# The-African-Research-Collective/karanta-ocr

Hardware: AMD Instinct MI355X
Metric: pages_per_sec (higher is better)
Workload: dtype bf16; 1 GPU; Qwen2-VL-2B bf16 greedy, batch=8 synthetic 1024x1024 pages per GPU, max_pixels=1003520 (grid 70x70, 1225 image tokens), prompt P=1394 tokens, T_out=1024 (ignore_eos), random-init weights; global_batch=8, parallelism=dp1, decode=hipGraph replay

## Files before the change

karanta_ocr_amd/_lib.py:

```python
from __future__ import annotations

import ctypes as C
import os
from typing import Optional

_HERE = os.path.dirname(os.path.abspath(__file__))
LIB_PATH = os.path.join(_HERE, "libkaranta_hip.so")

c_p = C.c_void_p
i32, i64, f32 = C.c_int, C.c_int64, C.c_float


class KarantaHipError(RuntimeError):
    pass


SIGNATURES = {
    "kr_version": [],
    "kr_last_error": [],
    "kr_device_info": [i32, C.c_char_p, C.POINTER(i32), C.POINTER(C.c_size_t)],
    "kr_set_device": [i32],
    "kr_stream_synchronize": [c_p],
    "kr_stream_create_cu_mask": [C.POINTER(c_p), i32],
    "kr_stream_create_cu_range": [C.POINTER(c_p), i32, i32],
# ... 94 lines not shown
    return C.byref(NarrowOpts(zero_ptr or None, int(zero_bytes), 1 if atomic_out else 0, int(part_rows)))

class Dec32(C.Structure):
    _fields_ = [("xp", c_p), ("w_packed", c_p), ("w_scale", c_p), ("bias", c_p), ("residual", c_p), ("ldr", C.c_int64),
                ("out", c_p), ("out_f32", c_p), ("ldc", C.c_int64), ("M", C.c_int32), ("N", C.c_int32), ("K", C.c_int32),
                ("waves_ref", C.c_int32), ("ksplit", C.c_int32), ("atomic_out", C.c_int32), ("tiles_per_wg", C.c_int32),
                ("group_split", C.c_int32), ("reserved0", C.c_int32), ("zero_ptr", c_p), ("zero_bytes", C.c_uint64),
                ("cs_table", c_p), ("cs_stride", C.c_int32), ("prompt_len", c_p), ("ctx_len", c_p),
                ("q_out", c_p), ("kcache", c_p), ("vtcache", c_p), ("heads", C.c_int32), ("kv_heads", C.c_int32), ("s_max", C.c_int32)]


ABI_MAJOR = 4
DEC_OUT_XP = 0x100
ADJ_CAP = 320
EPI_NONE, EPI_QUICK_GELU, EPI_GELU_ERF, EPI_SILU_MUL, EPI_SILU_MUL8 = 0, 1, 2, 3, 4
DEC_PLAIN, DEC_SILU, DEC_ROPE_KV, DEC_ARGMAX, DEC_SILU8 = 0, 1, 2, 3, 4


class _Lib:
    def __init__(self, path: str):
        if not os.path.exists(path):
            raise KarantaHipError(
                f"{path} not found: build it with `python -m karanta_ocr_amd.build` "
                "(the MI355X engine has no CPU fallback)")
        import torch

        try:
            self._dll = C.CDLL(path, mode=C.RTLD_GLOBAL)
        except OSError as e:
            raise KarantaHipError(f"cannot load {path}: {e}") from e
        self.path = path
        for name, argtypes in SIGNATURES.items():
            try:
                fn = getattr(self._dll, name)
            except AttributeError as e:
                raise KarantaHipError(f"{path} does not export {name}") from e
            fn.argtypes = argtypes
            fn.restype = _RESTYPES.get(name, C.c_int)
            if name in ("kr_version", "kr_last_error"):
                setattr(self, name, fn)
            else:
                setattr(self, name, self._checked(name, fn))
        if self.kr_version() // 100 != ABI_MAJOR:
            raise KarantaHipError(f"{path} reports kr_version() = {self.kr_version()}, this binding is written against ABI major "
                                  f"{ABI_MAJOR} (include/karanta_hip.h): rebuild with `python -m karanta_ocr_amd.build`")
        self.experiments = hasattr(self._dll, "kr_oproj_heads")
        for name, argtypes in EXPERIMENT_SIGNATURES.items():
            if self.experiments:
                fn = getattr(self._dll, name)
                fn.argtypes, fn.restype = argtypes, C.c_int
                setattr(self, name, self._checked(name, fn))
            else:
                setattr(self, name, self._absent(name))

    @staticmethod
    def _absent(name):
        def call(*_):
            raise KarantaHipError(f"{name} is an experiment entry point (include/karanta_hip_experiments.h): this library was built "
                                  "without -DKR_EXPERIMENTS (csrc/tools/build_variant.py; load it through KARANTA_HIP_LIB)")
        call.__name__ = name
        return call

    def _checked(self, name, fn):
        def call(*args):
            rc = fn(*args)
            if rc != 0:
                msg = self._dll.kr_last_error()
                raise KarantaHipError(f"{name} -> {rc}: {msg.decode() if msg else ''}")
            return rc

        call.__name__ = name
        call.raw = fn
        return call


_LIB: Optional[_Lib] = None


def lib() -> _Lib:
    global _LIB
    if _LIB is None:
        _LIB = _Lib(os.environ.get("KARANTA_HIP_LIB", LIB_PATH))
    return _LIB


def ptr(t) -> int:
    return 0 if t is None else t.data_ptr()
```

karanta_ocr_amd/csrc/kr_decode.hip:

```cpp
#include "kr_decode_common.h"

namespace {

struct DecLinArgs {
    const kr_bf16* x; int64_t ldx;
    const kr_bf16* wp;
    const kr_bf16* bias;
    const kr_bf16* norm_w; float norm_eps;
    const kr_bf16* residual; int64_t ldr;
    kr_bf16* out; float* out_f32; int64_t ldc;
    int M, N, K, ksplit;
    int groups;
    float* ws; int* counters;
    const float* attn_ws; int attn_split;
    int xmode;
    const float* cs_table;
    const int32_t* prompt_len; int cs_stride;
    const int32_t* ctx_len;
    kr_bf16* q_out; kr_bf16* kcache; kr_bf16* vtcache;
    int heads, kv_heads, s_max;
    float* amax_val; int32_t* amax_idx;
    int wide_blocks, wide_waves;
    const float* part_in; kr_bf16* x_out; int64_t ldxo;
    const float* w_scale;
    float* x_out_f32; int64_t ldxf;
    kr_bf16* wide_x_out; int64_t wide_ldxo;
    int x_is_f32;
    const char* pf_ptr; int64_t pf_bytes; int pf_blocks;
    int part_rows;
    int n_part;
    int part_atomic;
    float* zero_ptr; int zero_n16;
    int out_xp;
};

template <int NT, int EPI, int WAVES>
__global__ void __launch_bounds__(WAVES * 64) dec_linear_kernel(const DecLinArgs a) {
    extern __shared__ __attribute__((aligned(16))) char smem[];
    constexpr int U = (WAVES == 16 ? 4 : 8) / NT;
    constexpr int NTHR = WAVES * 64;
    const int tid = threadIdx.x, lane = tid & 63;
    const int wave = __builtin_amdgcn_readfirstlane(tid >> 6);
    const int fr = lane & 15, fg = lane >> 4;
    const int ks = blockIdx.y;
    const int M = a.M, K = a.K;
    const int nchunks = K >> 6, ntiles = a.N >> 4;
    const int cpb = (nchunks + a.ksplit - 1) / a.ksplit;
    const int cb0 = min(ks * cpb, nchunks), cb1 = min(cb0 + cpb, nchunks);
    const int nblk = cb1 - cb0;
    const int per = (nblk + WAVES - 1) / WAVES;
    const int c0 = min(cb0 + wave * per, cb1), c1 = min(c0 + per, cb1);

    int tile[NT];
    const kr_bf16* wp[NT];
    bf16x8 wbuf[U][NT][2];
    auto set_item = [&](int g) {
        if (EPI == DEPI_ROPE_KV) {
            tile[0] = (g >> 2) * 8 + (g & 3);
            tile[NT - 1] = tile[0] + 4;
        } else {
#pragma unroll
            for (int t = 0; t < NT; ++t) tile[t] = g * NT + t;
        }
#pragma unroll
        for (int t = 0; t < NT; ++t) {
            const int tt = tile[t] < ntiles ? tile[t] : ntiles - 1;
            wp[t] = a.wp + ((int64_t)tt * nchunks) * 1024 + lane * 8;
        }
#pragma unroll
        for (int u = 0; u < U; ++u) {
            const int c = c0 + u;
            if (c < c1) {
#pragma unroll
                for (int t = 0; t < NT; ++t) {
                    wbuf[u][t][0] = ld8_nt(wp[t] + (int64_t)c * 1024);
                    wbuf[u][t][1] = ld8_nt(wp[t] + (int64_t)c * 1024 + 512);
                }
            }
        }
    };
    int g = blockIdx.x;
    set_item(g);

    const bool xlds = a.xmode != 0;
    const int xrow = nblk * 128 + 16;
    float* red = reinterpret_cast<float*>(smem + (xlds ? ((M * xrow + 127) & ~127) : 0));
// ... 801 lines not shown
        KR_CHECK_ARG(tiles_per_wave <= 5, "kr_linear_decode_wide: %d tiles over %d x %d waves is more than 5 tiles per wave", a.N >> 4,
                     blocks, waves);
        KR_CHECK_ARG(!a.x_is_f32 && !a.bias && !a.residual, "kr_linear_decode_wide: K-halves take bf16 x, no bias / residual");
        const size_t lds = (size_t)32 * (28 * 64 * 2 + 16);
        auto fn = tiles_per_wave <= 2 ? &dec_wide_kh_kernel<EPI, W8, true> : &dec_wide_kh_kernel<EPI, W8, false>;
        static KrPerDeviceOnce attr;
        if (attr.need()) {
            KR_CHECK_HIP(hipFuncSetAttribute(reinterpret_cast<const void*>(&dec_wide_kh_kernel<EPI, W8, true>),
                                             hipFuncAttributeMaxDynamicSharedMemorySize, 160 * 1024));
            KR_CHECK_HIP(hipFuncSetAttribute(reinterpret_cast<const void*>(&dec_wide_kh_kernel<EPI, W8, false>),
                                             hipFuncAttributeMaxDynamicSharedMemorySize, 160 * 1024));
        }
        fn<<<blocks, 512, lds, kr_hs(s)>>>(a.x, a.wp, a.norm_w, a.ldx, a.M, a.N, a.wide_blocks, a.wide_waves, a.norm_eps, a);
        KR_CHECK_LAUNCH();
        return KR_OK;
    } else {
        kr_set_error("kr_linear_decode_wide: M=%d > 16 at K = 3584 is built for the SILU8 and ARGMAX modes", a.M);
        return KR_ERR_ARG;
    }
}

template <int EPI, int NCH, bool W8>
int launch_wide_w(DecLinArgs& a, int blocks, int waves, kr_stream s) {
    if (a.M > 16) {
        if constexpr (NCH == 56) {
            return launch_wide_kh<EPI, W8>(a, blocks, waves, s);
        } else {
            return launch_wide_m<EPI, NCH, W8, 2>(a, blocks, waves, s);
        }
    }
    return launch_wide_m<EPI, NCH, W8, 1>(a, blocks, waves, s);
}

template <int EPI, int NCH>
int launch_wide_n(DecLinArgs& a, int blocks, int waves, kr_stream s) {
    return a.w_scale ? launch_wide_w<EPI, NCH, true>(a, blocks, waves, s) : launch_wide_w<EPI, NCH, false>(a, blocks, waves, s);
}

template <int EPI>
int launch_wide(DecLinArgs& a, int blocks, int waves, kr_stream s) {
    switch (a.K >> 6) {
        case 24: return launch_wide_n<EPI, 24>(a, blocks, waves, s);
        case 32: return launch_wide_n<EPI, 32>(a, blocks, waves, s);
        case 56: return launch_wide_n<EPI, 56>(a, blocks, waves, s);
        default: return launch_wide_n<EPI, 0>(a, blocks, waves, s);
    }
}

template <int NCH> struct NarrowCfg { static constexpr int RL = 8; };
template <> struct NarrowCfg<24> { static constexpr int RL = 3; };
template <> struct NarrowCfg<32> { static constexpr int RL = 4; };
template <> struct NarrowCfg<56> { static constexpr int RL = 7; };

template <int NT, int EPI, int WAVES, int NCH, int PKS, bool NORM, int U, bool W8, int MT>
__global__ void __launch_bounds__(WAVES * 64) dec_narrow_kernel(const kr_bf16* hx, const kr_bf16* hwp, const kr_bf16* hnorm_w, const float* hpart_in,
                                                                int64_t hldx, int hM, int hN, int hK, int hcpb, float hnorm_eps,
                                                                int hprows, const DecLinArgs a) {
    extern __shared__ __attribute__((aligned(16))) char smem[];
    using WC = WChunk<W8>;
    constexpr int RL = NarrowCfg<NCH>::RL;
    constexpr bool FULL = NCH != 0;
    const int tid = threadIdx.x, lane = tid & 63;
    const int wave = __builtin_amdgcn_readfirstlane(tid >> 6);
    const int fr = lane & 15, fg = lane >> 4;
    const int g = blockIdx.x, ks = blockIdx.y;
    if (KR_EXP && a.pf_blocks > 0 && (int)blockIdx.x >= (int)gridDim.x - a.pf_blocks) {
        const int pb = blockIdx.x - ((int)gridDim.x - a.pf_blocks);
        const int64_t n16 = a.pf_bytes >> 4, stride = (int64_t)a.pf_blocks * (WAVES * 64);
        const u32x4* p = reinterpret_cast<const u32x4*>(a.pf_ptr);
        u32x4 acc = {0u, 0u, 0u, 0u};
        int64_t i = (int64_t)pb * (WAVES * 64) + threadIdx.x;
        for (; i + 15 * stride < n16; i += 16 * stride) {
            u32x4 v[16];
#pragma unroll
            for (int k = 0; k < 16; ++k) v[k] = p[i + k * stride];
#pragma unroll
            for (int k = 0; k < 16; ++k) acc ^= v[k];
        }
        for (; i < n16; i += stride) acc ^= p[i];
        asm volatile("" ::"v"(acc[0] ^ acc[1] ^ acc[2] ^ acc[3]));
        return;
    }
    const int M = hM, K = hK;
    const int nchunks = NCH ? NCH : (K >> 6), ntiles = hN >> 4, kc = K >> 3;
    const int cpb = hcpb;
    const int cb0 = min(ks * cpb, nchunks), cb1 = min(cb0 + cpb, nchunks);
    const int nblk = cb1 - cb0;
    const int c0 = cb0 + (wave * nblk) / WAVES, c1 = cb0 + ((wave + 1) * nblk) / WAVES;
    const int xrow = nblk * 128 + 16;
    float* red = reinterpret_cast<float*>(smem + (NORM ? ((M * xrow + 127) & ~127) : 0));

    int tile[NT];
    if (EPI == DEPI_ROPE_KV) {
        tile[0] = (g >> 2) * 8 + (g & 3);
        tile[NT - 1] = tile[0] + 4;
    } else {
#pragma unroll
        for (int t = 0; t < NT; ++t) tile[t] = g * NT + t;
    }
    const char* wp[NT];
#pragma unroll
    for (int t = 0; t < NT; ++t)
        wp[t] = reinterpret_cast<const char*>(hwp) + ((int64_t)min(tile[t], ntiles - 1) * nchunks) * WC::BYTES + lane * 16;
    int rb[MT];
#pragma unroll
    for (int mt = 0; mt < MT; ++mt) rb[mt] = min(fr + 16 * mt, M - 1);

    bf16x8 xv[NORM ? RL : 1], nwv[NORM ? RL : 1];
    f32x4 pv[PKS ? PKS : 1][NORM ? RL : 1][2];
    bf16x8 xf[NORM ? 1 : U][MT][2];
    const char* xg[MT];
#pragma unroll
    for (int mt = 0; mt < MT; ++mt) xg[mt] = reinterpret_cast<const char*>(hx + (int64_t)rb[mt] * hldx);
    if (NORM) {
        const int b = wave < M ? wave : 0;
#pragma unroll
        for (int i = 0; i < RL; ++i) {
            const int c = lane + i * 64;
            if (FULL || c < kc) {
                xv[i] = ld8(hx + (int64_t)b * hldx + c * 8);
#pragma unroll
                for (int k = 0; k < PKS; ++k) {
                    const float* pp = hpart_in + ((int64_t)k * hprows + b) * K + c * 8;
                    pv[k][i][0] = *reinterpret_cast<const f32x4*>(pp);
                    pv[k][i][1] = *reinterpret_cast<const f32x4*>(pp + 4);
                }
                nwv[i] = ld8(hnorm_w + c * 8);
            }
        }
    } else {
#pragma unroll
        for (int u = 0; u < U; ++u) {
            const int c = min(max(min(c0 + u, c1 - 1), cb0), nchunks - 1);
#pragma unroll
            for (int mt = 0; mt < MT; ++mt) {
                xf[u][mt][0] = *reinterpret_cast<const bf16x8*>(xg[mt] + c * 128 + WC::x_byte(0, fg));
                xf[u][mt][1] = *reinterpret_cast<const bf16x8*>(xg[mt] + c * 128 + WC::x_byte(1, fg));
            }
        }
    }
    int pos[MT], plen[MT];
#pragma unroll
    for (int mt = 0; mt < MT; ++mt) {
        pos[mt] = plen[mt] = 0;
        if (EPI == DEPI_ROPE_KV) {
            pos[mt] = a.ctx_len[rb[mt]];
            plen[mt] = a.prompt_len[rb[mt]];
        }
    }
    WC wbuf[U][NT];
#pragma unroll
    for (int u = 0; u < U; ++u) {
        const int c = min(max(min(c0 + u, c1 - 1), cb0), nchunks - 1);
#pragma unroll
        for (int t = 0; t < NT; ++t) wbuf[u][t].load(wp[t], c);
    }
    __builtin_amdgcn_sched_barrier(0);
    if (a.zero_ptr) {
        const int zgx = (int)gridDim.x - (KR_EXP ? a.pf_blocks : 0);
        const int zstep = zgx * (int)gridDim.y * (WAVES * 64);
        for (int zi = ((int)blockIdx.y * zgx + (int)blockIdx.x) * (WAVES * 64) + tid; zi < a.zero_n16; zi += zstep)
            reinterpret_cast<f32x4*>(a.zero_ptr)[zi] = (f32x4){0.f, 0.f, 0.f, 0.f};
    }

    if constexpr (NORM) {
        auto norm_row = [&](const int b, bf16x8 (&xr)[RL], const bf16x8 (&nw)[RL]) {
            float ss = 0.f;
#pragma unroll
            for (int i = 0; i < RL; ++i) {
                if (FULL || lane + i * 64 < kc) {
#pragma unroll
                    for (int j = 0; j < 8; ++j) ss += bf2f(xr[i][j]) * bf2f(xr[i][j]);
                }
            }
            ss = wave_sum(ss);
            const float rs = rsqrtf(ss / (float)K + hnorm_eps);
#pragma unroll
            for (int i = 0; i < RL; ++i) {
                const int c = lane + i * 64;
                if ((FULL || c < kc) && c >= cb0 * 8 && c < cb1 * 8) {
                    bf16x8 o;
#pragma unroll
                    for (int j = 0; j < 8; ++j) o[j] = f2bf(bf2f(nw[i][j]) * bfround(bf2f(xr[i][j]) * rs));
                    *reinterpret_cast<bf16x8*>(smem + b * xrow + (c - cb0 * 8) * 16) = o;
                }
            }
        };
        if (PKS) {
#pragma unroll
            for (int i = 0; i < RL; ++i) {
                if (FULL || lane + i * 64 < kc) {
#pragma unroll
                    for (int j = 0; j < 8; ++j) {
                        float v = bf2f(xv[i][j]);
#pragma unroll
                        for (int k = 0; k < PKS; ++k) v += pv[k][i][j >> 2][j & 3];
                        xv[i][j] = f2bf(v);
                    }
                    if (g == 0 && ks == 0 && wave < M)
                        *reinterpret_cast<bf16x8*>(a.x_out + (int64_t)wave * a.ldxo + (lane + i * 64) * 8) = xv[i];
                }
            }
        }
        if (KR_EXP && a.x_out_f32 && g == 0 && ks == 0 && wave < M) {
#pragma unroll
            for (int i = 0; i < RL; ++i) {
                if (FULL || lane + i * 64 < kc) {
                    float* xo = a.x_out_f32 + (int64_t)wave * a.ldxf + (lane + i * 64) * 8;
                    *reinterpret_cast<f32x4*>(xo) = (f32x4){bf2f(xv[i][0]), bf2f(xv[i][1]), bf2f(xv[i][2]), bf2f(xv[i][3])};
                    *reinterpret_cast<f32x4*>(xo + 4) = (f32x4){bf2f(xv[i][4]), bf2f(xv[i][5]), bf2f(xv[i][6]), bf2f(xv[i][7])};
                }
            }
        }
        if (wave < M) norm_row(wave, xv, nwv);
        for (int b = wave + WAVES; b < M; b += WAVES) {
            bf16x8 v[RL];
#pragma unroll
            for (int i = 0; i < RL; ++i) {
                const int c = lane + i * 64;
                if (FULL || c < kc) {
                    v[i] = ld8(hx + (int64_t)b * hldx + c * 8);
                    if (PKS) {
                        float f[8];
#pragma unroll
                        for (int j = 0; j < 8; ++j) f[j] = bf2f(v[i][j]);
#pragma unroll
                        for (int k = 0; k < PKS; ++k) {
                            const float* pp = hpart_in + ((int64_t)k * hprows + b) * K + c * 8;
                            const f32x4 p0 = *reinterpret_cast<const f32x4*>(pp), p1 = *reinterpret_cast<const f32x4*>(pp + 4);
#pragma unroll
                            for (int j = 0; j < 4; ++j) {
                                f[j] += p0[j];
                                f[4 + j] += p1[j];
                            }
                        }
#pragma unroll
                        for (int j = 0; j < 8; ++j) v[i][j] = f2bf(f[j]);
                        if (g == 0 && ks == 0) *reinterpret_cast<bf16x8*>(a.x_out + (int64_t)b * a.ldxo + c * 8) = v[i];
                    }
                    if (KR_EXP && a.x_out_f32 && g == 0 && ks == 0) {
                        float* xo = a.x_out_f32 + (int64_t)b * a.ldxf + c * 8;
                        *reinterpret_cast<f32x4*>(xo) = (f32x4){bf2f(v[i][0]), bf2f(v[i][1]), bf2f(v[i][2]), bf2f(v[i][3])};
                        *reinterpret_cast<f32x4*>(xo + 4) = (f32x4){bf2f(v[i][4]), bf2f(v[i][5]), bf2f(v[i][6]), bf2f(v[i][7])};
                    }
                }
            }
            norm_row(b, v, nwv);
        }
        __syncthreads();
    }
    float csv[MT][8];
    bf16x4 bias0 = {}, bias1 = {};
#pragma unroll
    for (int mt = 0; mt < MT; ++mt)
#pragma unroll
        for (int j = 0; j < 8; ++j) csv[mt][j] = 0.f;
    if (EPI == DEPI_ROPE_KV) {
        const int i0 = (tile[0] & 7) * 16 + fg * 4;
#pragma unroll
        for (int mt = 0; mt < MT; ++mt) {
            const float* cs = a.cs_table + ((int64_t)rb[mt] * a.cs_stride + (pos[mt] - plen[mt])) * 128;
            const f32x4 cv = *reinterpret_cast<const f32x4*>(cs + i0), sv = *reinterpret_cast<const f32x4*>(cs + 64 + i0);
#pragma unroll
            for (int j = 0; j < 4; ++j) {
                csv[mt][j] = cv[j];
                csv[mt][4 + j] = sv[j];
            }
        }
        bias0 = *reinterpret_cast<const bf16x4*>(a.bias + tile[0] * 16 + fg * 4);
        bias1 = *reinterpret_cast<const bf16x4*>(a.bias + tile[NT - 1] * 16 + fg * 4);
    }

    bf16x4 res_pre[MT][NT], bias_pre[NT];
    if (EPI == DEPI_PLAIN) {
#pragma unroll
        for (int t = 0; t < NT; ++t) {
            const int n = min(tile[t], ntiles - 1) * 16 + fg * 4;
            bias_pre[t] = *reinterpret_cast<const bf16x4*>(a.bias ? a.bias + n : hx);
#pragma unroll
            for (int mt = 0; mt < MT; ++mt)
                res_pre[mt][t] = *reinterpret_cast<const bf16x4*>(a.residual ? a.residual + (int64_t)rb[mt] * a.ldr + n : hx);
        }
    }

    const char* xl[MT];
#pragma unroll
    for (int mt = 0; mt < MT; ++mt) xl[mt] = smem + rb[mt] * xrow;
    f32x4 acc[MT][NT];
#pragma unroll
    for (int mt = 0; mt < MT; ++mt)
#pragma unroll
        for (int t = 0; t < NT; ++t) acc[mt][t] = (f32x4){0.f, 0.f, 0.f, 0.f};
    for (int cc = c0; cc < c1; cc += U) {
#pragma unroll
        for (int u = 0; u < U; ++u) {
            const int c = cc + u;
            if (c < c1) {
                bf16x8 x0[MT], x1[MT];
#pragma unroll
                for (int mt = 0; mt < MT; ++mt) {
                    if (NORM) {
                        x0[mt] = *reinterpret_cast<const bf16x8*>(xl[mt] + (c - cb0) * 128 + WC::x_byte(0, fg));
                        x1[mt] = *reinterpret_cast<const bf16x8*>(xl[mt] + (c - cb0) * 128 + WC::x_byte(1, fg));
                    } else {
                        x0[mt] = xf[u][mt][0];
                        x1[mt] = xf[u][mt][1];
                    }
                }
#pragma unroll
                for (int t = 0; t < NT; ++t) {
                    const bf16x8 w0 = wbuf[u][t].frag(0), w1 = wbuf[u][t].frag(1);
#pragma unroll
                    for (int mt = 0; mt < MT; ++mt) {
                        acc[mt][t] = __builtin_amdgcn_mfma_f32_16x16x32_bf16(w0, x0[mt], acc[mt][t], 0, 0, 0);
                        acc[mt][t] = __builtin_amdgcn_mfma_f32_16x16x32_bf16(w1, x1[mt], acc[mt][t], 0, 0, 0);
                    }
                }
                const int cn = c + U;
                if (cn < c1) {
                    if (!NORM) {
#pragma unroll
                        for (int mt = 0; mt < MT; ++mt) {
                            xf[u][mt][0] = *reinterpret_cast<const bf16x8*>(xg[mt] + cn * 128 + WC::x_byte(0, fg));
                            xf[u][mt][1] = *reinterpret_cast<const bf16x8*>(xg[mt] + cn * 128 + WC::x_byte(1, fg));
                        }
                    }
#pragma unroll
                    for (int t = 0; t < NT; ++t) wbuf[u][t].load(wp[t], cn);
                }
            }
        }
    }
    auto epilogue = [&](const int mt, f32x4 (&sum)[NT]) {
        const int b = fr + 16 * mt;
        if (b >= M) return;
#pragma unroll
        for (int t = 0; t < NT; ++t) apply_w_scale(a.w_scale, min(tile[t], ntiles - 1) * 16 + fg * 4, sum[t]);
        if (EPI == DEPI_ROPE_KV) {
            const int hh = tile[0] >> 3;
            const int i0 = (tile[0] & 7) * 16 + fg * 4;
            float lo[4], hi[4];
#pragma unroll
            for (int j = 0; j < 4; ++j) {
                lo[j] = bfround(sum[0][j] + bf2f(bias0[j]));
                hi[j] = bfround(sum[NT - 1][j] + bf2f(bias1[j]));
            }
            if (hh < a.heads + a.kv_heads) {
                bf16x4 o0, o1;
#pragma unroll
                for (int j = 0; j < 4; ++j) {
                    o0[j] = f2bf(lo[j] * csv[mt][j] - hi[j] * csv[mt][4 + j]);
                    o1[j] = f2bf(hi[j] * csv[mt][j] + lo[j] * csv[mt][4 + j]);
                }
                kr_bf16* dst = hh < a.heads
                                   ? a.q_out + ((int64_t)b * a.heads + hh) * 128
                                   : a.kcache + (((int64_t)b * a.kv_heads + (hh - a.heads)) * a.s_max + pos[mt]) * 128;
                *reinterpret_cast<bf16x4*>(dst + i0) = o0;
                *reinterpret_cast<bf16x4*>(dst + 64 + i0) = o1;
            } else {
                const int kvh = hh - a.heads - a.kv_heads;
                kr_bf16* vt = a.vtcache + (((int64_t)b * a.kv_heads + kvh) * (a.s_max >> 6) + (pos[mt] >> 6)) * (128 * 64) + kr_vt_off(0, pos[mt] & 63, 128);
#pragma unroll
                for (int j = 0; j < 4; ++j) {
                    vt[(i0 + j) * 32] = __builtin_bit_cast(kr_bf16, f2bf(lo[j]));
                    vt[(64 + i0 + j) * 32] = __builtin_bit_cast(kr_bf16, f2bf(hi[j]));
                }
            }
            return;
        }
#pragma unroll
        for (int t = 0; t < NT; ++t) {
            if (tile[t] >= ntiles) continue;
            const int n = tile[t] * 16 + fg * 4;
            if (EPI == DEPI_PARTIAL) {
                if (a.part_atomic) {
                    float* acc = a.out_f32 + (int64_t)b * a.ldc + n;
#pragma unroll
                    for (int j = 0; j < 4; ++j) atomicAdd(acc + j, sum[t][j]);
                } else {
                    *reinterpret_cast<f32x4*>(a.out_f32 + ((int64_t)ks * M + b) * a.ldc + n) = sum[t];
                }
                continue;
            }
            float v[4];
#pragma unroll
            for (int j = 0; j < 4; ++j) v[j] = sum[t][j];
            if (a.bias) {
                const bf16x4 bv = EPI == DEPI_PLAIN ? bias_pre[t] : *reinterpret_cast<const bf16x4*>(a.bias + n);
#pragma unroll
                for (int j = 0; j < 4; ++j) v[j] += bf2f(bv[j]);
            }
            if (a.residual) {
                const bf16x4 rv = EPI == DEPI_PLAIN ? res_pre[mt][t]
                                                    : *reinterpret_cast<const bf16x4*>(a.residual + (int64_t)b * a.ldr + n);
#pragma unroll
                for (int j = 0; j < 4; ++j) v[j] += bf2f(rv[j]);
            }
            if (a.out_f32) {
                *reinterpret_cast<f32x4*>(a.out_f32 + (int64_t)b * a.ldc + n) = (f32x4){v[0], v[1], v[2], v[3]};
            } else {
                bf16x4 o;
#pragma unroll
                for (int j = 0; j < 4; ++j) o[j] = f2bf(v[j]);
                *reinterpret_cast<bf16x4*>(a.out + (int64_t)b * a.ldc + n) = o;
            }
        }
    };
#pragma unroll
    for (int mt = 0; mt < MT; ++mt) {
        if (mt > 0) __syncthreads();
#pragma unroll
        for (int t = 0; t < NT; ++t) *reinterpret_cast<f32x4*>(red + ((wave * NT + t) * 64 + lane) * 4) = acc[mt][t];
        __syncthreads();
        if (wave == 0) {
            f32x4 sum[NT];
#pragma unroll
            for (int t = 0; t < NT; ++t) {
                f32x4 half[2];
#pragma unroll
                for (int hfi = 0; hfi < 2; ++hfi) {
                    half[hfi] = (f32x4){0.f, 0.f, 0.f, 0.f};
#pragma unroll
                    for (int w = hfi * (WAVES / 2); w < (hfi + 1) * (WAVES / 2); ++w) {
                        const f32x4 p = *reinterpret_cast<const f32x4*>(red + ((w * NT + t) * 64 + lane) * 4);
#pragma unroll
                        for (int j = 0; j < 4; ++j) half[hfi][j] += p[j];
                    }
                }
#pragma unroll
                for (int j = 0; j < 4; ++j) sum[t][j] = half[0][j] + half[1][j];
            }
            epilogue(mt, sum);
        }
    }
}

template <int NT, int EPI, int WAVES, int NCH, int PKS, bool NORM, int U, bool W8, int MT>
int launch_narrow_m(DecLinArgs& a, int groups, kr_stream s) {
    const int nchunks = a.K >> 6, cpb = (nchunks + a.ksplit - 1) / a.ksplit;
    const size_t xbytes = NORM ? (((size_t)a.M * (cpb * 128 + 16) + 127) & ~(size_t)127) : 0;
    const size_t lds = xbytes + (size_t)WAVES * NT * 256 * 4;
    KR_CHECK_ARG(lds <= 160 * 1024, "kr_linear_decode_narrow: M=%d K=%d needs %zu bytes of LDS", a.M, a.K, lds);
    auto fn = &dec_narrow_kernel<NT, EPI, WAVES, NCH, PKS, NORM, U, W8, MT>;
    static KrPerDeviceOnce attr;
    if (attr.need()) {
        KR_CHECK_HIP(hipFuncSetAttribute(reinterpret_cast<const void*>(fn), hipFuncAttributeMaxDynamicSharedMemorySize, 160 * 1024));
    }
    KR_CHECK_ARG(a.pf_blocks == 0 || a.ksplit == 1, "kr_linear_decode_narrow: prefetch workgroups need ksplit 1");
    fn<<<dim3(groups + a.pf_blocks, a.ksplit), WAVES * 64, lds, kr_hs(s)>>>(a.x, a.wp, a.norm_w, a.part_in, a.ldx, a.M, a.N, a.K, cpb,
                                                                            a.norm_eps, a.part_rows > 0 ? a.part_rows : a.M, a);
    KR_CHECK_LAUNCH();
    return KR_OK;
}

template <int NT, int EPI, int WAVES, int NCH, int PKS, bool NORM, int U, bool W8>
int launch_narrow_w(DecLinArgs& a, int groups, kr_stream s) {
    if (a.M > 16) {
        if constexpr (WAVES == 8 && NCH != 56) {
            return launch_narrow_m<NT, EPI, WAVES, NCH, PKS, NORM, U, W8, 2>(a, groups, s);
        } else {
            kr_set_error("kr_linear_decode_narrow: M=%d > 16 needs 8-wave workgroups and K != 3584", a.M);
            return KR_ERR_ARG;
        }
    }
    return launch_narrow_m<NT, EPI, WAVES, NCH, PKS, NORM, U, W8, 1>(a, groups, s);
}

template <int NT, int EPI, int WAVES, int NCH, int PKS, bool NORM, int U>
int launch_narrow_u(DecLinArgs& a, int groups, kr_stream s) {
    return a.w_scale ? launch_narrow_w<NT, EPI, WAVES, NCH, PKS, NORM, U, true>(a, groups, s)
                     : launch_narrow_w<NT, EPI, WAVES, NCH, PKS, NORM, U, false>(a, groups, s);
}

inline int narrow_share(const DecLinArgs& a, int waves) {
    const int nchunks = a.K >> 6, cpb = (nchunks + a.ksplit - 1) / a.ksplit;
    return (cpb + waves - 1) / waves;
}

template <int EPI, int WAVES>
int launch_narrow_direct(DecLinArgs& a, int groups, kr_stream s) {
    const int share = narrow_share(a, WAVES);
    if constexpr (EPI == DEPI_PARTIAL) {
        const char* e = getenv("KARANTA_NARROW_NT2");
        const bool nt2 = e ? atoi(e) != 0 : groups >= 192;
        if (nt2 && (groups & 1) == 0 && (a.M <= 16 || WAVES == 8)) {
            if constexpr (WAVES == 16) return launch_narrow_u<2, EPI, WAVES, 0, 0, false, 3>(a, groups / 2, s);
            else return launch_narrow_u<2, EPI, WAVES, 0, 0, false, 5>(a, groups / 2, s);
        }
    }
    if (share <= 3) return launch_narrow_u<1, EPI, WAVES, 0, 0, false, 3>(a, groups, s);
    if constexpr (WAVES == 16) {
        return launch_narrow_u<1, EPI, WAVES, 0, 0, false, 5>(a, groups, s);
    } else {
        if (share <= 5) return launch_narrow_u<1, EPI, WAVES, 0, 0, false, 5>(a, groups, s);
        return launch_narrow_u<1, EPI, WAVES, 0, 0, false, 8>(a, groups, s);
    }
}

template <int NT, int EPI, int NCH, int PKS>
int launch_narrow_norm_u(DecLinArgs& a, int groups, kr_stream s) {
    if (narrow_share(a, 8) <= 3) return launch_narrow_u<NT, EPI, 8, NCH, PKS, true, 3>(a, groups, s);
    return launch_narrow_u<NT, EPI, 8, NCH, PKS, true, 8 / NT>(a, groups, s);
}
// ... 237 lines not shown
    KR_CHECK_ARG(x && w_packed, "kr_linear_decode_wide: null pointer");
    KR_CHECK_ARG(M >= 1 && M <= 32, "kr_linear_decode_wide: M=%d must be in 1..32", M);
    KR_CHECK_ARG(N > 0 && N % 16 == 0 && K > 0 && K % 512 == 0 && K <= 4096,
                 "kr_linear_decode_wide: N=%d K=%d (N%%16, K%%512, K<=4096)", N, K);
    KR_CHECK_ARG(ldx >= K && (ldx & 7) == 0, "kr_linear_decode_wide: ldx");
    KR_CHECK_ARG(blocks > 0 && waves >= 1 && waves <= 8, "kr_linear_decode_wide: blocks=%d waves=%d", blocks, waves);
    DecLinArgs a{};
    a.x_is_f32 = x_is_f32 ? 1 : 0; a.wide_x_out = x_out; a.wide_ldxo = ldxo;
    a.x = x; a.ldx = ldx; a.wp = reinterpret_cast<const kr_bf16*>(w_packed); a.w_scale = w_scale; a.bias = bias;
    a.norm_w = norm_w; a.norm_eps = norm_eps;
    a.residual = residual; a.ldr = ldr; a.out = out; a.out_f32 = out_f32; a.ldc = ldc;
    a.M = M; a.N = N; a.K = K; a.ksplit = 1; a.amax_val = amax_val; a.amax_idx = amax_idx;
    a.wide_blocks = blocks; a.wide_waves = waves;
    if (mode & KR_DEC_OUT_XP) {
        KR_CHECK_ARG((mode & ~KR_DEC_OUT_XP) == DEPI_SILU8 && M > 16 && (N / 2) % 64 == 0 && ((uintptr_t)out & 15) == 0,
                     "kr_linear_decode_wide: KR_DEC_OUT_XP is for SILU8 at 17..32 rows, N/2 %% 64 == 0");
        a.out_xp = 1;
        mode &= ~KR_DEC_OUT_XP;
    }
    switch (mode) {
        case DEPI_PLAIN:
            KR_CHECK_ARG((out || out_f32) && ldc >= N && (ldc & 3) == 0 && (!residual || (ldr & 3) == 0), "kr_linear_decode_wide: PLAIN output");
            return launch_wide<DEPI_PLAIN>(a, blocks, waves, s);
        case DEPI_SILU8:
            KR_CHECK_ARG(out && ldc >= N / 2 && (ldc & 3) == 0, "kr_linear_decode_wide: SILU8 output");
            return launch_wide<DEPI_SILU8>(a, blocks, waves, s);
        case DEPI_ARGMAX:
            KR_CHECK_ARG(amax_val && amax_idx && (!out_f32 || ldc >= N), "kr_linear_decode_wide: ARGMAX pointers");
            return launch_wide<DEPI_ARGMAX>(a, blocks, waves, s);
        default:
            kr_set_error("kr_linear_decode_wide: mode %d not supported (PLAIN, SILU8, ARGMAX)", mode);
            return KR_ERR_ARG;
    }
}

extern "C" int kr_linear_decode_wide(int mode, const kr_bf16* x, int64_t ldx, const kr_bf16* w_packed, const kr_bf16* bias,
                                     const kr_bf16* norm_w, float norm_eps, const kr_bf16* residual, int64_t ldr,
                                     kr_bf16* out, float* out_f32, int64_t ldc, int M, int N, int K, int blocks, int waves,
                                     float* amax_val, int32_t* amax_idx, kr_stream s) {
    return wide_impl(mode, x, ldx, w_packed, nullptr, bias, norm_w, norm_eps, residual, ldr, out, out_f32, ldc, M, N, K, blocks,
                     waves, amax_val, amax_idx, s);
}

extern "C" int kr_linear_decode_wide_fp8(int mode, const kr_bf16* x, int64_t ldx, const uint8_t* w_packed_fp8,
                                         const float* w_scale, const kr_bf16* bias, const kr_bf16* norm_w, float norm_eps,
                                         const kr_bf16* residual, int64_t ldr, kr_bf16* out, float* out_f32, int64_t ldc,
                                         int M, int N, int K, int blocks, int waves, float* amax_val, int32_t* amax_idx,
                                         kr_stream s) {
    KR_CHECK_ARG(w_scale, "kr_linear_decode_wide_fp8: w_scale is NULL");
    return wide_impl(mode, x, ldx, w_packed_fp8, w_scale, bias, norm_w, norm_eps, residual, ldr, out, out_f32, ldc, M, N, K,
                     blocks, waves, amax_val, amax_idx, s);
}

static int narrow_impl(int mode, const kr_bf16* x, int64_t ldx, const float* part_in, int n_part_in,
                                       kr_bf16* x_out, int64_t ldxo, const void* w_packed, const float* w_scale, const kr_bf16* bias,
                                       const kr_bf16* norm_w, float norm_eps, const kr_bf16* residual, int64_t ldr,
                                       kr_bf16* out, float* out_f32, int64_t ldc, int M, int N, int K, int waves, int ksplit,
                                       const float* cs_table, int cs_stride, const int32_t* prompt_len, const int32_t* ctx_len,
                                       kr_bf16* q_out, kr_bf16* kcache, kr_bf16* vtcache, int heads, int kv_heads, int s_max,
                                       const kr_narrow_opts* opts, kr_stream s, float* x_out_f32 = nullptr, int64_t ldxf = 0,
                                       const void* pf_ptr = nullptr, size_t pf_bytes = 0, int pf_blocks = 0) {
    KR_CHECK_ARG(x && w_packed, "kr_linear_decode_narrow: null pointer");
    const kr_narrow_opts o = opts ? *opts : kr_narrow_opts{};
    KR_CHECK_ARG((o.zero_ptr || o.zero_bytes == 0) && ((uintptr_t)o.zero_ptr & 15) == 0 && (o.zero_bytes & 15) == 0 && o.zero_bytes < (1u << 30),
                 "kr_linear_decode_narrow: opts zero range");
    KR_CHECK_ARG(o.part_rows >= 0 && o.part_rows <= 32, "kr_linear_decode_narrow: opts part_rows=%d", o.part_rows);
    KR_CHECK_ARG(M >= 1 && M <= 32, "kr_linear_decode_narrow: M=%d must be in 1..32", M);
    KR_CHECK_ARG(N > 0 && N % 16 == 0 && K > 0 && K % 64 == 0, "kr_linear_decode_narrow: N=%d K=%d (N%%16, K%%64)", N, K);
    KR_CHECK_ARG(ldx >= K && (ldx & 7) == 0, "kr_linear_decode_narrow: ldx");
    KR_CHECK_ARG(waves == 8 || waves == 16, "kr_linear_decode_narrow: waves=%d (8 or 16)", waves);
    KR_CHECK_ARG(ksplit >= 1 && ksplit <= 8 && ksplit <= (K >> 6), "kr_linear_decode_narrow: ksplit=%d", ksplit);
    KR_CHECK_ARG(!norm_w || K <= 4096, "kr_linear_decode_narrow: fused RMSNorm supports K <= 4096");
    KR_CHECK_ARG(!part_in || (norm_w && (n_part_in == 1 || n_part_in == 2) && x_out && x_out != x && ldxo >= K && (ldxo & 7) == 0),
                 "kr_linear_decode_narrow: partial sums need the norm prologue, 1 or 2 slabs and a separate x_out");
    DecLinArgs a{};
    a.x = x; a.ldx = ldx; a.wp = reinterpret_cast<const kr_bf16*>(w_packed); a.w_scale = w_scale; a.bias = bias;
    a.norm_w = norm_w; a.norm_eps = norm_eps;
    a.residual = residual; a.ldr = ldr; a.out = out; a.out_f32 = out_f32; a.ldc = ldc;
    a.M = M; a.N = N; a.K = K; a.ksplit = ksplit;
    a.part_in = part_in; a.x_out = x_out; a.ldxo = ldxo;
    a.x_out_f32 = x_out_f32; a.ldxf = ldxf;
    a.part_rows = o.part_rows;
    a.n_part = part_in ? n_part_in : 0;
    a.zero_ptr = o.zero_bytes ? o.zero_ptr : nullptr; a.zero_n16 = (int)(o.zero_bytes >> 4); a.part_atomic = o.atomic_out ? 1 : 0;
    KR_CHECK_ARG(!a.part_atomic || (ksplit == 2 && mode == DEPI_PLAIN), "kr_linear_decode_narrow: atomic_out is for ksplit 2 (order-free sum)");
    KR_CHECK_ARG(a.part_rows == 0 || (part_in && a.part_rows >= M), "kr_linear_decode_narrow: part rows %d < M %d", a.part_rows, M);
    if (KR_EXP && pf_blocks > 0) {
        KR_CHECK_ARG(ksplit == 1 && pf_ptr && ((uintptr_t)pf_ptr & 15) == 0 && pf_blocks <= 1024, "kr_linear_decode_narrow_pf: bad args");
        a.pf_ptr = reinterpret_cast<const char*>(pf_ptr); a.pf_bytes = (int64_t)pf_bytes; a.pf_blocks = pf_bytes >= 16 ? pf_blocks : 0;
    }
    a.cs_table = cs_table; a.cs_stride = cs_stride; a.prompt_len = prompt_len; a.ctx_len = ctx_len;
    a.q_out = q_out; a.kcache = kcache; a.vtcache = vtcache;
    a.heads = heads; a.kv_heads = kv_heads; a.s_max = s_max;
    const int ntiles = N >> 4;
    switch (mode) {
        case DEPI_PLAIN:
            KR_CHECK_ARG(ldc >= N && (ldc & 3) == 0 && (!residual || (ldr & 3) == 0), "kr_linear_decode_narrow: PLAIN ldc / ldr");
            if (ksplit > 1) {
                KR_CHECK_ARG(out_f32 && !out && !bias && !residual && !norm_w,
                             "kr_linear_decode_narrow: split-K writes f32 slabs only (no bias / residual / norm)");
                return waves == 16 ? launch_narrow_direct<DEPI_PARTIAL, 16>(a, ntiles, s)
                                   : launch_narrow_direct<DEPI_PARTIAL, 8>(a, ntiles, s);
            }
            KR_CHECK_ARG(out || out_f32, "kr_linear_decode_narrow: PLAIN output");
            if (norm_w) return launch_narrow_norm<1, DEPI_PLAIN>(a, ntiles, s);
            return waves == 16 ? launch_narrow_direct<DEPI_PLAIN, 16>(a, ntiles, s)
                               : launch_narrow_direct<DEPI_PLAIN, 8>(a, ntiles, s);
        case DEPI_ROPE_KV:
            KR_CHECK_ARG(bias && cs_table && prompt_len && ctx_len && q_out && kcache && vtcache && cs_stride > 0,
                         "kr_linear_decode_narrow: ROPE_KV pointers");
            KR_CHECK_ARG(N == (heads + 2 * kv_heads) * 128 && s_max % 64 == 0 && ksplit == 1,
                         "kr_linear_decode_narrow: ROPE_KV needs head_dim 128, ksplit 1");
            if (!norm_w) {
                KR_CHECK_ARG(!part_in && waves == 8, "kr_linear_decode_narrow: ROPE_KV without a norm takes no partial sums, 8 waves");
                if (narrow_share(a, 8) <= 3) return launch_narrow_u<2, DEPI_ROPE_KV, 8, 0, 0, false, 3>(a, ntiles / 2, s);
                return launch_narrow_u<2, DEPI_ROPE_KV, 8, 0, 0, false, 5>(a, ntiles / 2, s);
            }
            return launch_narrow_norm<2, DEPI_ROPE_KV>(a, ntiles / 2, s);
        default:
            kr_set_error("kr_linear_decode_narrow: mode %d not supported (PLAIN, ROPE_KV)", mode);
            return KR_ERR_ARG;
    }
}

extern "C" int kr_linear_decode_narrow(int mode, const kr_bf16* x, int64_t ldx, const float* part_in, int n_part_in,
                                       kr_bf16* x_out, int64_t ldxo, const kr_bf16* w_packed, const kr_bf16* bias,
                                       const kr_bf16* norm_w, float norm_eps, const kr_bf16* residual, int64_t ldr,
                                       kr_bf16* out, float* out_f32, int64_t ldc, int M, int N, int K, int waves, int ksplit,
                                       const float* cs_table, int cs_stride, const int32_t* prompt_len, const int32_t* ctx_len,
                                       kr_bf16* q_out, kr_bf16* kcache, kr_bf16* vtcache, int heads, int kv_heads, int s_max,
                                       const kr_narrow_opts* opts, kr_stream s) {
    return narrow_impl(mode, x, ldx, part_in, n_part_in, x_out, ldxo, w_packed, nullptr, bias, norm_w, norm_eps, residual, ldr, out,
                       out_f32, ldc, M, N, K, waves, ksplit, cs_table, cs_stride, prompt_len, ctx_len, q_out, kcache, vtcache,
                       heads, kv_heads, s_max, opts, s);
}
// ... 194 lines not shown
```

Before: 6.159 pages/s.

## Reorder narrow decode kernel prologue to overlap loads and defer side writes

Restructures the narrow decode GEMV prologue. It moves the RoPE position and cos/sin table loads after the matmul, and the x_out/x_out_f32 copies and zero-fill after the epilogue. It also pre-warms the kernarg scalar cache with s_load_dword and narrows ldx to int. The intent is to shorten the critical path before weight streaming and MFMA, letting latency-bound loads overlap compute. It also adds optional cycle-counter stamps behind a compile flag for profiling; moving the zero-fill and x_out writes later risks ordering assumptions with consumers.

After: 6.211 pages/s (median of 6 runs). About the same (+0.8%).

```diff
diff --git a/karanta_ocr_amd/_lib.py b/karanta_ocr_amd/_lib.py
--- a/karanta_ocr_amd/_lib.py
+++ b/karanta_ocr_amd/_lib.py
@@ -170,6 +170,11 @@
                 setattr(self, name, self._checked(name, fn))
             else:
                 setattr(self, name, self._absent(name))
+        self.narrow_stamps = hasattr(self._dll, "kr_narrow_stamps")
+        if self.narrow_stamps:
+            fn = self._dll.kr_narrow_stamps
+            fn.argtypes, fn.restype = [c_p], C.c_int
+            self.kr_narrow_stamps = self._checked("kr_narrow_stamps", fn)
 
     @staticmethod
     def _absent(name):
diff --git a/karanta_ocr_amd/csrc/kr_decode.hip b/karanta_ocr_amd/csrc/kr_decode.hip
--- a/karanta_ocr_amd/csrc/kr_decode.hip
+++ b/karanta_ocr_amd/csrc/kr_decode.hip
@@ -32,6 +32,7 @@
     int part_atomic;
     float* zero_ptr; int zero_n16;
     int out_xp;
+    unsigned long long* stamps;
 };
 
 template <int NT, int EPI, int WAVES>
@@ -939,9 +940,19 @@
 template <> struct NarrowCfg<32> { static constexpr int RL = 4; };
 template <> struct NarrowCfg<56> { static constexpr int RL = 7; };
 
+#ifdef KR_NARROW_STAMPS
+constexpr bool KR_STAMPS = true;
+#define KR_STAMP_DECL unsigned long long stamp[8] = {}
+#define KR_STAMP(i) do { __builtin_amdgcn_sched_barrier(0); stamp[i] = __builtin_readcyclecounter(); __builtin_amdgcn_sched_barrier(0); } while (0)
+#else
+constexpr bool KR_STAMPS = false;
+#define KR_STAMP_DECL do { } while (0)
+#define KR_STAMP(i) do { } while (0)
+#endif
+
 template <int NT, int EPI, int WAVES, int NCH, int PKS, bool NORM, int U, bool W8, int MT>
 __global__ void __launch_bounds__(WAVES * 64) dec_narrow_kernel(const kr_bf16* hx, const kr_bf16* hwp, const kr_bf16* hnorm_w, const float* hpart_in,
-                                                                int64_t hldx, int hM, int hN, int hK, int hcpb, float hnorm_eps,
+                                                                int hldx, float hnorm_eps, int hM, int hN, int hK, int hcpb,
                                                                 int hprows, const DecLinArgs a) {
     extern __shared__ __attribute__((aligned(16))) char smem[];
     using WC = WChunk<W8>;
@@ -951,6 +962,8 @@
     const int wave = __builtin_amdgcn_readfirstlane(tid >> 6);
     const int fr = lane & 15, fg = lane >> 4;
     const int g = blockIdx.x, ks = blockIdx.y;
+    KR_STAMP_DECL;
+    KR_STAMP(0);
     if (KR_EXP && a.pf_blocks > 0 && (int)blockIdx.x >= (int)gridDim.x - a.pf_blocks) {
         const int pb = blockIdx.x - ((int)gridDim.x - a.pf_blocks);
         const int64_t n16 = a.pf_bytes >> 4, stride = (int64_t)a.pf_blocks * (WAVES * 64);
@@ -1026,15 +1039,6 @@
             }
         }
     }
-    int pos[MT], plen[MT];
-#pragma unroll
-    for (int mt = 0; mt < MT; ++mt) {
-        pos[mt] = plen[mt] = 0;
-        if (EPI == DEPI_ROPE_KV) {
-            pos[mt] = a.ctx_len[rb[mt]];
-            plen[mt] = a.prompt_len[rb[mt]];
-        }
-    }
     WC wbuf[U][NT];
 #pragma unroll
     for (int u = 0; u < U; ++u) {
@@ -1042,14 +1046,14 @@
 #pragma unroll
         for (int t = 0; t < NT; ++t) wbuf[u][t].load(wp[t], c);
     }
+    unsigned warm[(sizeof(DecLinArgs) + 63) / 64];
+    {
+        const char* kargs = (const char*)__builtin_amdgcn_kernarg_segment_ptr();
+#pragma unroll
+        for (int i = 0; i < (int)(sizeof(warm) / sizeof(warm[0])); ++i)
+            asm volatile("s_load_dword %0, %1, %2" : "=s"(warm[i]) : "s"(kargs), "s"(64 + 64 * i));
+    }
     __builtin_amdgcn_sched_barrier(0);
-    if (a.zero_ptr) {
-        const int zgx = (int)gridDim.x - (KR_EXP ? a.pf_blocks : 0);
-        const int zstep = zgx * (int)gridDim.y * (WAVES * 64);
-        for (int zi = ((int)blockIdx.y * zgx + (int)blockIdx.x) * (WAVES * 64) + tid; zi < a.zero_n16; zi += zstep)
-            reinterpret_cast<f32x4*>(a.zero_ptr)[zi] = (f32x4){0.f, 0.f, 0.f, 0.f};
-    }
-
     if constexpr (NORM) {
         auto norm_row = [&](const int b, bf16x8 (&xr)[RL], const bf16x8 (&nw)[RL]) {
             float ss = 0.f;
@@ -1062,6 +1066,10 @@
             }
             ss = wave_sum(ss);
             const float rs = rsqrtf(ss / (float)K + hnorm_eps);
+            if (KR_STAMPS && b < WAVES) {
+                asm volatile("" ::"v"(rs));
+                KR_STAMP(2);
+            }
 #pragma unroll
             for (int i = 0; i < RL; ++i) {
                 const int c = lane + i * 64;
@@ -1084,21 +1092,11 @@
                         for (int k = 0; k < PKS; ++k) v += pv[k][i][j >> 2][j & 3];
                         xv[i][j] = f2bf(v);
                     }
-                    if (g == 0 && ks == 0 && wave < M)
-                        *reinterpret_cast<bf16x8*>(a.x_out + (int64_t)wave * a.ldxo + (lane + i * 64) * 8) = xv[i];
-                }
-            }
-        }
-        if (KR_EXP && a.x_out_f32 && g == 0 && ks == 0 && wave < M) {
-#pragma unroll
-            for (int i = 0; i < RL; ++i) {
-                if (FULL || lane + i * 64 < kc) {
-                    float* xo = a.x_out_f32 + (int64_t)wave * a.ldxf + (lane + i * 64) * 8;
-                    *reinterpret_cast<f32x4*>(xo) = (f32x4){bf2f(xv[i][0]), bf2f(xv[i][1]), bf2f(xv[i][2]), bf2f(xv[i][3])};
-                    *reinterpret_cast<f32x4*>(xo + 4) = (f32x4){bf2f(xv[i][4]), bf2f(xv[i][5]), bf2f(xv[i][6]), bf2f(xv[i][7])};
-                }
-            }
-        }
+                }
+            }
+        }
+        if (KR_STAMPS) asm volatile("" ::"v"(xv[RL - 1]));
+        KR_STAMP(1);
         if (wave < M) norm_row(wave, xv, nwv);
         for (int b = wave + WAVES; b < M; b += WAVES) {
             bf16x8 v[RL];
@@ -1134,30 +1132,26 @@
             }
             norm_row(b, v, nwv);
         }
-        __syncthreads();
-    }
-    float csv[MT][8];
+    }
+    int pos[MT], plen[MT];
     bf16x4 bias0 = {}, bias1 = {};
 #pragma unroll
-    for (int mt = 0; mt < MT; ++mt)
-#pragma unroll
-        for (int j = 0; j < 8; ++j) csv[mt][j] = 0.f;
+    for (int mt = 0; mt < MT; ++mt) {
+        pos[mt] = plen[mt] = 0;
+        if (EPI == DEPI_ROPE_KV) {
+            pos[mt] = a.ctx_len[rb[mt]];
+            plen[mt] = a.prompt_len[rb[mt]];
+        }
+    }
     if (EPI == DEPI_ROPE_KV) {
-        const int i0 = (tile[0] & 7) * 16 + fg * 4;
-#pragma unroll
-        for (int mt = 0; mt < MT; ++mt) {
-            const float* cs = a.cs_table + ((int64_t)rb[mt] * a.cs_stride + (pos[mt] - plen[mt])) * 128;
-            const f32x4 cv = *reinterpret_cast<const f32x4*>(cs + i0), sv = *reinterpret_cast<const f32x4*>(cs + 64 + i0);
-#pragma unroll
-            for (int j = 0; j < 4; ++j) {
-                csv[mt][j] = cv[j];
-                csv[mt][4 + j] = sv[j];
-            }
-        }
         bias0 = *reinterpret_cast<const bf16x4*>(a.bias + tile[0] * 16 + fg * 4);
         bias1 = *reinterpret_cast<const bf16x4*>(a.bias + tile[NT - 1] * 16 + fg * 4);
     }
-
+    KR_STAMP(7);
+    if constexpr (NORM) __syncthreads();
+#pragma unroll
+    for (int i = 0; i < (int)(sizeof(warm) / sizeof(warm[0])); ++i) asm volatile("s_waitcnt lgkmcnt(0)" ::"s"(warm[i]));
+    KR_STAMP(3);
     bf16x4 res_pre[MT][NT], bias_pre[NT];
     if (EPI == DEPI_PLAIN) {
 #pragma unroll
@@ -1218,6 +1212,26 @@
             }
         }
     }
+    float csv[MT][8];
+#pragma unroll
+    for (int mt = 0; mt < MT; ++mt)
+#pragma unroll
+        for (int j = 0; j < 8; ++j) csv[mt][j] = 0.f;
+    if (EPI == DEPI_ROPE_KV) {
+        const int i0 = (tile[0] & 7) * 16 + fg * 4;
+#pragma unroll
+        for (int mt = 0; mt < MT; ++mt) {
+            const float* cs = a.cs_table + ((int64_t)rb[mt] * a.cs_stride + (pos[mt] - plen[mt])) * 128;
+            const f32x4 cv = *reinterpret_cast<const f32x4*>(cs + i0), sv = *reinterpret_cast<const f32x4*>(cs + 64 + i0);
+#pragma unroll
+            for (int j = 0; j < 4; ++j) {
+                csv[mt][j] = cv[j];
+                csv[mt][4 + j] = sv[j];
+            }
+        }
+    }
+    if (KR_STAMPS) asm volatile("" ::"v"(acc[MT - 1][NT - 1]));
+    KR_STAMP(4);
     auto epilogue = [&](const int mt, f32x4 (&sum)[NT]) {
         const int b = fr + 16 * mt;
         if (b >= M) return;
@@ -1317,9 +1331,46 @@
 #pragma unroll
                 for (int j = 0; j < 4; ++j) sum[t][j] = half[0][j] + half[1][j];
             }
+            if (KR_STAMPS) asm volatile("" ::"v"(sum[NT - 1]));
+            if (mt == MT - 1) KR_STAMP(5);
             epilogue(mt, sum);
         }
     }
+    if constexpr (NORM && PKS > 0) {
+        if (g == 0 && ks == 0 && wave < M) {
+#pragma unroll
+            for (int i = 0; i < RL; ++i) {
+                if (FULL || lane + i * 64 < kc)
+                    *reinterpret_cast<bf16x8*>(a.x_out + (int64_t)wave * a.ldxo + (lane + i * 64) * 8) = xv[i];
+            }
+        }
+    }
+    if constexpr (NORM) {
+        if (KR_EXP && a.x_out_f32 && g == 0 && ks == 0 && wave < M) {
+#pragma unroll
+            for (int i = 0; i < RL; ++i) {
+                if (FULL || lane + i * 64 < kc) {
+                    float* xo = a.x_out_f32 + (int64_t)wave * a.ldxf + (lane + i * 64) * 8;
+                    *reinterpret_cast<f32x4*>(xo) = (f32x4){bf2f(xv[i][0]), bf2f(xv[i][1]), bf2f(xv[i][2]), bf2f(xv[i][3])};
+                    *reinterpret_cast<f32x4*>(xo + 4) = (f32x4){bf2f(xv[i][4]), bf2f(xv[i][5]), bf2f(xv[i][6]), bf2f(xv[i][7])};
+                }
+            }
+        }
+    }
+    if (a.zero_ptr) {
+        const int zgx = (int)gridDim.x - (KR_EXP ? a.pf_blocks : 0);
+        const int zstep = zgx * (int)gridDim.y * (WAVES * 64);
+        for (int zi = ((int)blockIdx.y * zgx + (int)blockIdx.x) * (WAVES * 64) + tid; zi < a.zero_n16; zi += zstep)
+            reinterpret_cast<f32x4*>(a.zero_ptr)[zi] = (f32x4){0.f, 0.f, 0.f, 0.f};
+    }
+    KR_STAMP(6);
+#ifdef KR_NARROW_STAMPS
+    if (a.stamps && lane == 0) {
+        unsigned long long* st = a.stamps + ((int64_t)((int)blockIdx.y * (int)gridDim.x + (int)blockIdx.x) * WAVES + wave) * 8;
+#pragma unroll
+        for (int i = 0; i < 8; ++i) st[i] = stamp[i];
+    }
+#endif
 }
 
 template <int NT, int EPI, int WAVES, int NCH, int PKS, bool NORM, int U, bool W8, int MT>
@@ -1334,8 +1385,9 @@
         KR_CHECK_HIP(hipFuncSetAttribute(reinterpret_cast<const void*>(fn), hipFuncAttributeMaxDynamicSharedMemorySize, 160 * 1024));
     }
     KR_CHECK_ARG(a.pf_blocks == 0 || a.ksplit == 1, "kr_linear_decode_narrow: prefetch workgroups need ksplit 1");
-    fn<<<dim3(groups + a.pf_blocks, a.ksplit), WAVES * 64, lds, kr_hs(s)>>>(a.x, a.wp, a.norm_w, a.part_in, a.ldx, a.M, a.N, a.K, cpb,
-                                                                            a.norm_eps, a.part_rows > 0 ? a.part_rows : a.M, a);
+    KR_CHECK_ARG(a.ldx < (int64_t)1 << 31, "kr_linear_decode_narrow: ldx");
+    fn<<<dim3(groups + a.pf_blocks, a.ksplit), WAVES * 64, lds, kr_hs(s)>>>(a.x, a.wp, a.norm_w, a.part_in, (int)a.ldx, a.norm_eps, a.M, a.N, a.K,
+                                                                            cpb, a.part_rows > 0 ? a.part_rows : a.M, a);
     KR_CHECK_LAUNCH();
     return KR_OK;
 }
@@ -1679,6 +1731,14 @@
                      blocks, waves, amax_val, amax_idx, s);
 }
 
+#ifdef KR_NARROW_STAMPS
+static unsigned long long* g_narrow_stamps = nullptr;
+extern "C" int kr_narrow_stamps(unsigned long long* stamps) {
+    g_narrow_stamps = stamps;
+    return KR_OK;
+}
+#endif
+
 static int narrow_impl(int mode, const kr_bf16* x, int64_t ldx, const float* part_in, int n_part_in,
                                        kr_bf16* x_out, int64_t ldxo, const void* w_packed, const float* w_scale, const kr_bf16* bias,
                                        const kr_bf16* norm_w, float norm_eps, const kr_bf16* residual, int64_t ldr,
@@ -1708,6 +1768,9 @@
     a.part_in = part_in; a.x_out = x_out; a.ldxo = ldxo;
     a.x_out_f32 = x_out_f32; a.ldxf = ldxf;
     a.part_rows = o.part_rows;
+#ifdef KR_NARROW_STAMPS
+    a.stamps = g_narrow_stamps;
+#endif
     a.n_part = part_in ? n_part_in : 0;
     a.zero_ptr = o.zero_bytes ? o.zero_ptr : nullptr; a.zero_n16 = (int)(o.zero_bytes >> 4); a.part_atomic = o.atomic_out ? 1 : 0;
     KR_CHECK_ARG(!a.part_atomic || (ksplit == 2 && mode == DEPI_PLAIN), "kr_linear_decode_narrow: atomic_out is for ksplit 2 (order-free sum)");
```
